# saptadeb/botLab

Measured on AMD Instinct MI355X. Metric: SLAM steps/sec (map+MCL+A*), higher is better.
Workload: dtype int8 grid / f32 poses with f64 intermediates / int64 weights; 1 GPU; full SLAM step on 200x200 @5cm grid (continuing from the shipped, already built obstacle_slam_10mx10m_5cm map), 100000 particles, 290 rays, A* replan on; particles=100000, rays=290, pipeline_depth=14, planner_lanes=2, planner_batch=6, parallelism=single GPU, collective=none

## Files before the change

### botlab_amd/csrc/bl_mcl.hip

```cpp
#include <math.h>
#include <stdio.h>
#include <stdlib.h>
#include <string.h>
#include <new>

#include <hip/hip_ext.h>
#include "bl_internal.h"
#include "bl_mcl_finish.h"

#define MCL_LDS_RAYS 384
#define MCL_MIN_BLOCKS 512
#define MCL_WIN_SMALL_BYTES (64 * 1024)
#define MCL_WIN_MAX 208
#define MCL_WIN_MARGIN 24
#define SCAN_THREADS 256
#define SCAN_ITEMS 2
#define SCAN_TILE (SCAN_THREADS * SCAN_ITEMS)


struct bl_pf {
    bl_ctx* ctx;
    int N, lo, hi, n_local;
    float4* rec[2];
    bool rec_external;
    int cur;
    double* tile_partials;
    ss_rec* fin_recs;
    ss_wild* fin_wild;
    int fin_subs_cap;
    mclf_tab_elem* fin_tabs;
    unsigned long long* fin_sync;
    unsigned int fin_gen;
    int fin_last_nrec;
    unsigned long long* prefix;
    float4* parent;
    pf_state* state;
    double* partials;
    int partials_cap;
    bool use_lds;
    int last_blocks, last_tile;
    int last_main_blocks, last_main_particles, last_tail_tile;
    bool fused_finish, no_fused_finish, no_packed, no_balance, no_framed, no_window, no_fast_trig, no_mirror_reuse, no_stage_dma, no_stage_x4;
    int window_override;
    int cus;
    int split_log2_override;
    int block_override;
    bool debug;
    bool strict;
    void* strict_recs; double* strict_starts;
    bool uniform_now;
    bool prefix_is_strict;
    double w_floor;
    unsigned long long* block_sums;
    int scan_blocks;
    int32_t* dbg_idx;
    int32_t* dbg_like;
    float* d_noise;
    bl_particle_t* d_export;
    int64_t pose_utime, parent_utime;
    bl_pose_xyt_t prev_odom;
    bool action_initialized, moved;
    double rot1, trans, rot2, rot1Std, transStd, rot2Std;
    uint64_t noise_seed;
    uint32_t step;
    bool initialized;
    bool pending_end;
    int64_t pending_utime;
// ... 313 lines not shown
    const pf_state* state;
    float4* parent;
    double* partials;
    int32_t* dbg_idx;
    int32_t* dbg_like;
    const int8_t* cells;
    const int8_t* framed;
    int framed_stride;
    bl_frame frame;
    const float* ranges;
    const float* thetas;
    const int64_t* times;
    int64_t t_begin; double t_den;
    int R;
    int N, lo, n_local;
    double r;
    double M_inv;
    double rot1, trans, rot2, rot1Std, transStd, rot2Std;
    const float* noise;
    uint32_t seed_lo, seed_hi, step;
    int interp;
    int resample;
    int strict;
    int win_w, win_h;
    int split_log2;
    int pk_ok;
    int theta_simple;
    int fast_trig;
    int stage_dma;
    float max_range_cells;
    int main_blocks, main_particles;
    const struct mcl_shard_tab* sh;
    struct pf_recovery_dev* rc;
};
struct mcl_shard_tab { int world, block; const float4* src[BL_MAX_SHARDS]; const unsigned long long* prefix[BL_MAX_SHARDS]; };

struct pf_recovery_dev {
    double w_slow, w_fast, w_avg, p;
    uint32_t updates, primed;
    unsigned long long t;
    unsigned long long total_at_fold;
    unsigned long long injected_total;
    const uint32_t* list;
    uint32_t F, W, k0, k1;
    double ox, oy, mpc;
};
#define RC_CTR 0x72637679u

__device__ __forceinline__ float4 gl_pose(const uint32_t a[4], uint32_t b0, const uint32_t* list, uint32_t F, uint32_t W,
                                          double ox, double oy, double mpc)
{
    const uint32_t r = (uint32_t)__umul64hi(((unsigned long long)a[0] << 32) | a[1], (unsigned long long)F);
    const uint32_t cell = list[r];
    const uint32_t cx = cell % W, cy = cell / W;
    const double fx = (double)(a[2] >> 8) * 0x1p-24, fy = (double)(a[3] >> 8) * 0x1p-24, ft = (double)(b0 >> 8) * 0x1p-24;
    const float x = (float)(ox + ((double)cx + fx) * mpc);
    const float y = (float)(oy + ((double)cy + fy) * mpc);
    const float th = bl_wrap_to_pi((float)((2.0 * ft - 1.0) * BL_PI));
    return make_float4(x, y, th, __uint_as_float(1u));
}

__device__ __forceinline__ float4 mcl_src_at(const mcl_args& a, int i)
{
    if (a.sh) return a.sh->src[i / a.sh->block][i];
    return a.src[i];
}
// ... 32 lines not shown
            float sn, cs;                                                               \
            bl_sincosf_cells(wrap_to_pi_cells(pth_r - rt.y, theta_simple), &sn, &cs);                   \
            acc += SCORE_EXPR;                                                          \
        }                                                                               \
    } while (0)

#define MCL_RAY_LOOP_FAST_RANGE(PM, LO, HI, HW)                                         \
    do {                                                                                \
        const int rounds_ = ((HI) - (LO)) >> sl2;                                       \
        int off_ = ((LO) + sub) * 16;                                                   \
        for (int k_ = 0; k_ < rounds_; ++k_, off_ += split * 16) {                      \
            const float4 rt = *(const float4*)((const char*)s_ray + off_);              \
            short2_t E_, X_;                                                            \
            ray_cells_fast<HW>(start, a.frame.cpm, rt.x, pth_r, rt.y, pcs_, rt.z, rt.w, trig_k1, trig_kh2, E_, X_);   \
            acc += score_cells_pk(PM, S, E_, X_);                                       \
        }                                                                               \
        if ((off_ >> 4) < (HI)) {                                                       \
            const float4 rt = *(const float4*)((const char*)s_ray + off_);              \
            short2_t E_, X_;                                                            \
            ray_cells_fast<HW>(start, a.frame.cpm, rt.x, pth_r, rt.y, pcs_, rt.z, rt.w, trig_k1, trig_kh2, E_, X_);   \
            acc += score_cells_pk(PM, S, E_, X_);                                       \
        }                                                                               \
    } while (0)
#define MCL_RAY_LOOP_FAST(PM) do { if (hw_trig_) MCL_RAY_LOOP_FAST_RANGE(PM, 0, cnt, true); else MCL_RAY_LOOP_FAST_RANGE(PM, 0, cnt, false); } while (0)

__device__ __forceinline__ double readlane_f64(double v, int lane)
{
    const int lo = __builtin_amdgcn_readlane(__double2loint(v), lane), hi = __builtin_amdgcn_readlane(__double2hiint(v), lane);
    return __hiloint2double(hi, lo);
}

__device__ __forceinline__ int kary_pos(int lo, int hi, int step, int k) { return min(lo + (k + 1) * step - 1, hi); }

__device__ __forceinline__ bool resample_reaches(double T, unsigned long long v, bool strict)
{
    return strict ? T <= __longlong_as_double((long long)v) : T <= (double)v;
}

#define MCL_BRACKET_Q 1
#define MCL_BRACKET_WINDOW 64
template <int Q, class Prefix>
__device__ __forceinline__ void resample_bracket(const Prefix& prefix, int N, double T, bool active,
                                                 int lane, int* out_lo, int* out_hi, bool strict = false, int m = -1)
{
    *out_lo = 0; *out_hi = N - 1;
    const unsigned long long act = __builtin_amdgcn_ballot_w64(active);
    if (!act) return;
    const double T0 = readlane_f64(T, __ffsll((long long)act) - 1), T1 = readlane_f64(T, 63 - __clzll((long long)act));
    const int m0 = __builtin_amdgcn_readlane(m, __ffsll((long long)act) - 1);
    if (m0 >= 0) {
        const int g = m0 - 31 * MCL_BRACKET_WINDOW;
        if (g >= 0 && g + 63 * MCL_BRACKET_WINDOW < N) {
            const unsigned long long v = prefix[g + lane * MCL_BRACKET_WINDOW];
            const unsigned long long b0 = __builtin_amdgcn_ballot_w64(resample_reaches(T0, v, strict));
            const unsigned long long b1 = __builtin_amdgcn_ballot_w64(resample_reaches(T1, v, strict));
            if (b0 && !(b0 & 1ull) && b1) {
                const int f0 = __ffsll((long long)b0) - 1, f1 = __ffsll((long long)b1) - 1;
                *out_lo = g + (f0 - 1) * MCL_BRACKET_WINDOW + 1;
                *out_hi = g + f1 * MCL_BRACKET_WINDOW;
                return;
            }
        }
    }
    int lo0 = 0, hi0 = N - 1, lo1 = 0, hi1 = N - 1;
    for (int round = 0; round < 8 && (lo0 < hi0 || lo1 < hi1); ++round) {
        const int step0 = (hi0 - lo0 + 64 * Q) / (64 * Q), step1 = (hi1 - lo1 + 64 * Q) / (64 * Q);
        unsigned long long v0[Q], v1[Q];
#pragma unroll
        for (int u = 0; u < Q; ++u) {
            v0[u] = prefix[kary_pos(lo0, hi0, step0, 64 * u + lane)];
            v1[u] = prefix[kary_pos(lo1, hi1, step1, 64 * u + lane)];
        }
        int f0 = -1, f1 = -1;
#pragma unroll
        for (int u = Q - 1; u >= 0; --u) {
            const unsigned long long b0 = __builtin_amdgcn_ballot_w64(resample_reaches(T0, v0[u], strict));
            const unsigned long long b1 = __builtin_amdgcn_ballot_w64(resample_reaches(T1, v1[u], strict));
            if (b0) f0 = 64 * u + __ffsll((long long)b0) - 1;
            if (b1) f1 = 64 * u + __ffsll((long long)b1) - 1;
        }
        if (f0 < 0) lo0 = hi0;
        else { const int nl = f0 ? kary_pos(lo0, hi0, step0, f0 - 1) + 1 : lo0; hi0 = kary_pos(lo0, hi0, step0, f0); lo0 = nl; }
        if (f1 < 0) lo1 = hi1;
        else { const int nl = f1 ? kary_pos(lo1, hi1, step1, f1 - 1) + 1 : lo1; hi1 = kary_pos(lo1, hi1, step1, f1); lo1 = nl; }
    }
    if (lo0 == hi0 && lo1 == hi1) { *out_lo = lo0; *out_hi = lo1; }
}
template <class Prefix>
__device__ __forceinline__ void resample_bracket(const Prefix& prefix, int N, double T, bool active,
                                                 int lane, int* out_lo, int* out_hi, bool strict = false, int m = -1)
{
    resample_bracket<1>(prefix, N, T, active, lane, out_lo, out_hi, strict, m);
}

template <class Prefix>
__device__ __forceinline__ int resample_bisect(const Prefix& prefix, double T, int lo, int hi, bool strict = false)
{
    while (lo < hi) {
        const int mid = (lo + hi) >> 1;
        if (resample_reaches(T, prefix[mid], strict)) hi = mid; else lo = mid + 1;
    }
    return lo;
}

#define MCL_STAGE_ROWS 6
template <class SrcRow>
__device__ __forceinline__ void stage_rows(int* s_map32, int rows, int wq, int q_lo, int q_hi, int sw, int n_sw, int lane, SrcRow src_row)
{
    for (int q0 = 0; q0 < wq; q0 += 64) {
        const int q = q0 + lane;
        const bool qin = q < wq, qdata = q >= q_lo && q < q_hi;
        for (int r0 = sw; r0 < rows; r0 += n_sw * MCL_STAGE_ROWS) {
            int v[MCL_STAGE_ROWS];
#pragma unroll
            for (int u = 0; u < MCL_STAGE_ROWS; ++u) {
                const int ry = r0 + u * n_sw;
                v[u] = 0;
                if (ry < rows) {
                    const int* src = src_row(ry);
                    if (src != nullptr && qdata) v[u] = src[q - q_lo];
                }
            }
#pragma unroll
            for (int u = 0; u < MCL_STAGE_ROWS; ++u) {
                const int ry = r0 + u * n_sw;
                if (ry < rows && qin) s_map32[ry * wq + q] = v[u];
            }
        }
    }
}

#ifdef MCL_STAMPS
#define MCL_STAMP_SLOTS 12
__device__ unsigned long long g_mcl_stamps[4096 * MCL_STAMP_SLOTS];
#define MCL_STAMP(k) do { if (threadIdx.x == 0 && blockIdx.x < 4096) g_mcl_stamps[blockIdx.x * MCL_STAMP_SLOTS + (k)] = wall_clock64(); } while (0)
// ... 127 lines not shown
            const int wq = win.w >> 2, fq = a.framed_stride >> 2;
            const int* f32 = (const int*)(a.framed - MCL_FRAME * a.framed_stride - 4);
            const int* org = f32 + (size_t)(win.y0 + MCL_FRAME) * fq + ((win.x0 + 4) >> 2);
            if (wq <= 64 && a.stage_dma) {
                if (lane < wq)
                    for (int ry = sw; ry < win.h; ry += n_sw)
                        __builtin_amdgcn_global_load_lds((const __attribute__((address_space(1))) void*)(org + (size_t)ry * fq + lane),
                                                         (__attribute__((address_space(3))) void*)(s_map32 + ry * wq), 4, 0, 0);
            } else
            stage_rows(s_map32, win.h, wq, 0, wq, sw, n_sw, lane, [&](int ry) -> const int* { return org + (size_t)ry * fq; });
        }
    }

    MCL_STAMP_T(4, pw * 64);
#ifdef MCL_STAMPS
    if (wave >= pw) { asm volatile("s_waitcnt vmcnt(0)" ::: "memory"); }
    MCL_STAMP_T(9, pw * 64);
#endif
    double t_units = 0, t_x = 0, t_y = 0, t_s = 0, t_c = 0;
    float2 pcs_own = make_float2(2.0f, 0.0f);
    float pth_sin = 0.0f, pth_cos = 1.0f;
    int i = mp;
    bool injected = false;
    float4 s = make_float4(0.f, 0.f, 0.f, 0.f);
    float px = 0.f, py = 0.f, pth = 0.f, sx0 = 0.f, sy0 = 0.f;
    double rs_T = 0.0;
    int rs_lo = 0, rs_hi = a.N - 1;
    const mcl_prefix_view pview = {a.sh, a.prefix};
    const int uni_n = a.resample ? a.state->uni_n : 0;
    if (a.resample && (!shared_pro || wave < pw)) {
        if (pro_active) { rs_T = a.r + mp * a.M_inv; if (!a.strict && uni_n <= 0) rs_T *= a.state->S; }
        if (uni_n > 0) { }
        else if (a.sh) resample_bracket(pview, a.N, rs_T, pro_active, lane, &rs_lo, &rs_hi, a.strict != 0);
        else resample_bracket<MCL_BRACKET_Q>(a.prefix, a.N, rs_T, pro_active, lane, &rs_lo, &rs_hi, a.strict != 0, pro_active ? mp : -1);
    }
    MCL_STAMP(5);
    if (pro_active) {
        if (a.resample && uni_n > 0) i = uni_search(a.state, uni_n, rs_T, a.N);
        else if (a.resample) i = a.sh ? resample_bisect(pview, rs_T, rs_lo, rs_hi, a.strict != 0) : resample_bisect(a.prefix, rs_T, rs_lo, rs_hi, a.strict != 0);
        MCL_STAMP(6);
        if (REC) {
            const pf_recovery_dev& rc = *a.rc;
            uint32_t d[4];
            bl_philox4x32((uint32_t)mp, rc.updates, RC_CTR, 2u, rc.k0, rc.k1, d);
            injected = (unsigned long long)d[0] < rc.t;
            if (injected) {
                uint32_t w0[4], w1[4];
                bl_philox4x32((uint32_t)mp, rc.updates, RC_CTR, 0u, rc.k0, rc.k1, w0);
                bl_philox4x32((uint32_t)mp, rc.updates, RC_CTR, 1u, rc.k0, rc.k1, w1);
                s = gl_pose(w0, w1[0], rc.list, rc.F, rc.W, rc.ox, rc.oy, rc.mpc);
                i = -1;
            }
        }
        if (!injected)
        s = mcl_src_at(a, i);
        float n1, n2, n3;
        if (a.noise) {
            n1 = a.noise[3 * jp]; n2 = a.noise[3 * jp + 1]; n3 = a.noise[3 * jp + 2];
        } else {
            float z[3];
            philox_normals3((uint32_t)mp, a.step, a.seed_lo, a.seed_hi, z);
            n1 = (float)(a.rot1 + a.rot1Std * (double)z[0]);
            n2 = (float)(a.trans + a.transStd * (double)z[1]);
            n3 = (float)(a.rot2 + a.rot2Std * (double)z[2]);
        }
        const float head = s.z + n1;
// ... 496 lines not shown
    if (t >= (long long)n_local * 12) return;
    const int j = (int)(t / 12), d = (int)(t % 12);
    uint32_t v;
    if (d < 5) {
        const float4 r = rec[lo + j];
        v = d == 0 ? (uint32_t)((uint64_t)pose_utime >> 32) : d == 1 ? (uint32_t)pose_utime
          : __float_as_uint(d == 2 ? r.x : (d == 3 ? r.y : r.z));
    } else if (d < 10) {
        const float4 p = parent[j];
        v = d == 5 ? (uint32_t)((uint64_t)parent_utime >> 32) : d == 6 ? (uint32_t)parent_utime
          : __float_as_uint(d == 7 ? p.x : (d == 8 ? p.y : p.z));
    } else {
        const double w = (double)__float_as_uint(rec[lo + j].w) / state->S;
        const uint64_t b = (uint64_t)__double_as_longlong(w);
        v = d == 10 ? (uint32_t)(b >> 32) : (uint32_t)b;
    }
    out[t] = bl_bswap32(v);
}

__global__ void k_pf_set_pose(pf_state* state, bl_pose_xyt_t pose, int only_utime)
{
    if (only_utime) state->pose.utime = pose.utime;
    else state->pose = pose;
}

static int pf_alloc(bl_pf* pf)
{
    size_t N = pf->cap, n = pf->cap_local;
    if (!pf->rec[0]) {
        BL_HIP(hipMalloc((void**)&pf->rec[0], N * sizeof(float4)));
        BL_HIP(hipMalloc((void**)&pf->rec[1], N * sizeof(float4)));
    }
    BL_HIP(hipMalloc((void**)&pf->prefix, N * sizeof(unsigned long long)));
    BL_HIP(hipMalloc((void**)&pf->parent, n * sizeof(float4)));
    BL_HIP(hipMalloc((void**)&pf->state, sizeof(pf_state)));
    int blocks = (int)((n * 64 + 255) / 256) + 1;
    BL_HIP(hipMalloc((void**)&pf->partials, (size_t)blocks * 5 * sizeof(double)));
    pf->partials_cap = blocks;
    static bool attr_set = false;
    if (!attr_set) {
        const int big = 384 * 384;
        BL_HIP(hipFuncSetAttribute((const void*)k_mcl_main<0, 256, 2>, hipFuncAttributeMaxDynamicSharedMemorySize, big));
        BL_HIP(hipFuncSetAttribute((const void*)k_mcl_main<0, 512, 2>, hipFuncAttributeMaxDynamicSharedMemorySize, big));
        BL_HIP(hipFuncSetAttribute((const void*)k_mcl_main<0, 1024, 2>, hipFuncAttributeMaxDynamicSharedMemorySize, big));
        BL_HIP(hipFuncSetAttribute((const void*)k_mcl_finish, hipFuncAttributeMaxDynamicSharedMemorySize, MCLF_LDS_BYTES));
        attr_set = true;
    }
    pf->scan_blocks = (int)((N + SCAN_TILE - 1) / SCAN_TILE);
    BL_HIP(hipMalloc((void**)&pf->block_sums, (size_t)pf->scan_blocks * sizeof(unsigned long long)));
    BL_HIP(hipMalloc((void**)&pf->tile_partials, (size_t)pf->scan_blocks * 5 * sizeof(double)));
    pf->fin_subs_cap = (int)(N / MCLF_SUB) + 4 * (MCLF_WG / 64);
    BL_HIP(hipMalloc((void**)&pf->fin_recs, (size_t)2 * pf->fin_subs_cap * sizeof(ss_rec)));
    if (!getenv("BOTLAB_MCL_NO_WILD")) BL_HIP(hipMalloc((void**)&pf->fin_wild, (size_t)2 * pf->fin_subs_cap * sizeof(ss_wild)));
    BL_HIP(hipMalloc((void**)&pf->fin_tabs, (size_t)2 * MCLF_TSLOTS * MCLF_SUB * sizeof(mclf_tab_elem)));
    BL_HIP(hipMalloc((void**)&pf->fin_sync, MCLF_SYNC_WORDS * sizeof(unsigned long long)));
    BL_HIP(hipMemsetAsync(pf->fin_sync, 0, MCLF_SYNC_WORDS * sizeof(unsigned long long), pf->ctx->stream));
    BL_HIP(hipMalloc((void**)&pf->dbg_idx, n * sizeof(int32_t)));
    BL_HIP(hipMalloc((void**)&pf->dbg_like, n * sizeof(int32_t)));
    BL_HIP(hipMemsetAsync(pf->dbg_idx, 0, n * sizeof(int32_t), pf->ctx->stream));
    BL_HIP(hipMemsetAsync(pf->dbg_like, 0, n * sizeof(int32_t), pf->ctx->stream));
    BL_HIP(hipMemsetAsync(pf->state, 0, sizeof(pf_state), pf->ctx->stream));
    return BL_OK;
}

extern "C" int bl_pf_create(bl_ctx* ctx, int num_particles, int shard_lo, int shard_hi, bl_pf** out)
{
    BL_CHECK_ARG(ctx != nullptr && out != nullptr);
    BL_CHECK_ARG(num_particles > 1);
    BL_CHECK_ARG(shard_lo >= 0 && shard_lo < shard_hi && shard_hi <= num_particles);
    BL_HIP(hipSetDevice(ctx->device));
    bl_pf* pf = new bl_pf();
    memset((void*)pf, 0, sizeof(*pf));
    pf->ctx = ctx;
    pf->N = num_particles; pf->lo = shard_lo; pf->hi = shard_hi; pf->n_local = shard_hi - shard_lo;
    pf->cap = num_particles; pf->cap_local = pf->n_local; pf->ad_next = num_particles;
    {
        volatile double wsum = 0.0;
        for (int i = 0; i < num_particles; ++i) wsum = wsum + 0.001;
        pf->w_floor = 0.001 / wsum;
    }
    pf->noise_seed = 0x243F6A8885A308D3ull;
    pf->use_lds = getenv("BOTLAB_MCL_NO_LDS") == nullptr;
    pf->no_fused_finish = getenv("BOTLAB_MCL_NO_FUSED_FINISH") != nullptr;
    pf->no_packed = getenv("BOTLAB_MCL_NO_PACKED") != nullptr;
    pf->no_balance = getenv("BOTLAB_MCL_NO_BALANCE") != nullptr;
    pf->no_framed = getenv("BOTLAB_MCL_NO_FRAMED") != nullptr;
    pf->no_mirror_reuse = getenv("BOTLAB_MCL_NO_MIRROR_REUSE") != nullptr;
    pf->no_stage_dma = getenv("BOTLAB_MCL_NO_STAGE_DMA") != nullptr;
    pf->no_stage_x4 = getenv("BOTLAB_MCL_NO_STAGE_X4") != nullptr;
    pf->no_window = getenv("BOTLAB_MCL_NO_WINDOW") != nullptr;
    pf->no_fast_trig = getenv("BOTLAB_MCL_NO_FAST_TRIG") != nullptr;
    pf->window_override = getenv("BOTLAB_MCL_WINDOW") ? atoi(getenv("BOTLAB_MCL_WINDOW")) : 0;
    { int cus = 0; if (hipDeviceGetAttribute(&cus, hipDeviceAttributeMultiprocessorCount, ctx->device) == hipSuccess) pf->cus = cus; }
    pf->split_log2_override = getenv("BOTLAB_MCL_SPLIT_LOG2") ? atoi(getenv("BOTLAB_MCL_SPLIT_LOG2")) : -1;
    if (pf->split_log2_override > 6) pf->split_log2_override = 6;
    pf->block_override = getenv("BOTLAB_MCL_BLOCK") ? atoi(getenv("BOTLAB_MCL_BLOCK")) : 0;
    if (pf->block_override != 0 && pf->block_override != 256 && pf->block_override != 512 && pf->block_override != 1024) pf->block_override = 0;
    *out = pf;
    return BL_OK;
}

extern "C" void bl_pf_destroy(bl_pf* pf)
{
    if (!pf) return;
    (void)hipStreamSynchronize(pf->ctx->stream);
    if (!pf->rec_external) { if (pf->rec[0]) (void)hipFree(pf->rec[0]); if (pf->rec[1]) (void)hipFree(pf->rec[1]); }
    void* ptrs[] = {pf->fin_wild, pf->tile_partials, pf->fin_recs, pf->fin_tabs, pf->fin_sync, pf->prefix, pf->parent, pf->state, pf->partials, pf->block_sums, pf->dbg_idx, pf->dbg_like,
                    pf->d_noise, pf->d_export, pf->sh_xchg, pf->sh_tab, pf->sh_fin, pf->sh_flags, pf->sh_peers_dev, pf->strict_recs, pf->strict_starts,
                    pf->gl_tiles, pf->gl_list, pf->sp_parts, pf->sp_out, pf->rc_list, pf->rc_dev, pf->ad_table};
    for (void* p : ptrs) if (p) (void)hipFree(p);
    if (pf->ad_hcount) { (void)hipHostFree(pf->ad_hcount); (void)hipEventDestroy(pf->ad_ev); }
    delete pf->ad_wfloor;
    delete pf;
}

extern "C" int bl_pf_set_exchange_buffers(bl_pf* pf, void* d_rec0, void* d_rec1)
{
    BL_CHECK_ARG(pf != nullptr && d_rec0 && d_rec1);
    if (pf->prefix) { bl_set_error("exchange buffers must be set before the filter is initialised"); return BL_ERR_STATE; }
    pf->rec[0] = (float4*)d_rec0; pf->rec[1] = (float4*)d_rec1; pf->rec_external = true;
    return BL_OK;
}

extern "C" void* bl_pf_exchange_rec_ptr(bl_pf* pf) { return pf && pf->prefix ? (void*)pf->rec[pf->pending_end ? pf->cur ^ 1 : pf->cur] : nullptr; }
extern "C" const void* bl_pf_pose_device_ptr(bl_pf* pf) { return pf && pf->state ? (const void*)&pf->state->pose : nullptr; }

static double pf_w_floor(const bl_pf* pf)
{
    return (pf->N == pf->cap || !pf->ad_wfloor) ? pf->w_floor : (*pf->ad_wfloor)[pf->N];
}

static void pf_adaptive_fill(bl_pf* pf)
{
    if (pf->ad_pending) { (void)hipEventSynchronize(pf->ad_ev); pf->ad_pending = false; }
    pf->ad_next = pf->cap;
    if (pf->N == pf->cap) return;
    pf->N = pf->n_local = pf->hi = pf->cap;
    pf->scan_blocks = (pf->cap + SCAN_TILE - 1) / SCAN_TILE;
}

// ... 25 lines not shown
        }
    }
    hipLaunchKernelGGL(k_pf_cumulative_strict, dim3(1), dim3(64), 0, pf->ctx->stream, pf->rec[which], pf->N, pf->state, (double*)pf->prefix);
}

static int pf_finish_fill(bl_pf* pf, mcl_finish_args* f)
{
    if (f->tile <= 0 || f->tail_tile <= 0) return -1;
    f->gthreads = mclf_gthreads(pf->N);
    for (int attempt = 0; attempt < 2; ++attempt) {
        const int chunk = mclf_chunk(f->gthreads);
        if (f->tile <= chunk && (chunk % f->tile) == 0 && f->tail_tile <= chunk && (chunk % f->tail_tile) == 0) break;
        if (attempt == 1 || f->gthreads == MCLF_GT_LARGE) return -1;
        f->gthreads = MCLF_GT_LARGE;
    }
    const int groups = mclf_groups(*f);
    f->groups = groups;
    f->groups_wait = groups;
    if (((++pf->fin_gen) & 0xffu) == 0u) ++pf->fin_gen;
    f->tag = pf->fin_gen;
    const int nrec = groups * (f->gthreads >> 6);
    if (pf->sh_world <= 1 && nrec != pf->fin_last_nrec && (int64_t)nrec <= pf->fin_subs_cap) {
        if (hipMemsetAsync(pf->fin_recs, 0, (size_t)2 * pf->fin_subs_cap * sizeof(ss_rec), pf->ctx->stream) != hipSuccess) return -1;
        pf->fin_last_nrec = nrec;
    }
    f->sh = nullptr;
    f->uni_mode = pf_uni_mode(pf, false);
    f->w_floor = pf_w_floor(pf);
    f->wild = pf->sh_world > 1 ? nullptr : pf->fin_wild;
    f->no_trees = getenv("BOTLAB_MCL_NO_TREES") != nullptr ? 1 : 0;
    f->recs = pf->fin_recs;
    f->tabs = pf->fin_tabs;
    f->sync = pf->fin_sync;
    if (pf->sh_world > 1) return groups;
    if ((int64_t)groups * (f->gthreads >> 6) > pf->fin_subs_cap) return -1;
    return groups;
}

static int pf_scan(bl_pf* pf, int which, int write_pose, int64_t utime)
{
    bl_ctx* ctx = pf->ctx;
    hipEvent_t e0, e1;
    int rc = bl_timer_begin(ctx, BL_K_MCL_SCAN, &e0, &e1);
    if (rc) return rc;
    hipLaunchKernelGGL(k_scan_tile_sums, dim3(pf->scan_blocks), dim3(SCAN_THREADS), 0, ctx->stream, pf->rec[which], pf->N,
                       pf->block_sums, write_pose ? pf->tile_partials : (double*)nullptr);
    if (write_pose) {
        mcl_finish_args f;
        f.partials = pf->tile_partials; f.nblocks = pf->scan_blocks;
        f.rec = pf->rec[which]; f.N = pf->N;
        f.tile = SCAN_TILE; f.main_blocks = pf->scan_blocks; f.main_particles = pf->N; f.tail_tile = 1;
        f.prefix = pf->prefix; f.state = pf->state; f.utime = utime;
        const int groups = pf_finish_fill(pf, &f);
        if (groups < 0) { bl_set_error("internal: finish launch shape"); return BL_ERR_STATE; }
        hipLaunchKernelGGL(k_mcl_finish, dim3(MCLF_EXTRA_WGS + f.groups_wait), dim3(MCLF_WG), MCLF_LDS_BYTES, ctx->stream, f);
    } else {
        hipLaunchKernelGGL(k_scan_write_prefix, dim3(pf->scan_blocks), dim3(SCAN_THREADS), 0, ctx->stream, pf->rec[which], pf->N,
                           pf->block_sums, pf->scan_blocks, pf->prefix, pf->state, pf_uni_mode(pf, true), pf_w_floor(pf));
    }
    BL_HIP(hipGetLastError());
    pf_strict_cumulative(pf, which);
    return bl_timer_end(ctx, BL_K_MCL_SCAN, e0, e1);
}

static void pf_reset_action(bl_pf* pf)
{
    pf->action_initialized = false; pf->moved = false;
    pf->rot1 = pf->trans = pf->rot2 = 0;
    pf->step = 0;
    pf->pending_end = false;
}

extern "C" int bl_pf_init_at_pose(bl_pf* pf, const bl_pose_xyt_t* pose, uint64_t seed)
{
    BL_CHECK_ARG(pf != nullptr && pose != nullptr);
    BL_HIP(hipSetDevice(pf->ctx->device));
    if (!pf->prefix) { int rc = pf_alloc(pf); if (rc) return rc; }
    pf_adaptive_fill(pf);
    pf->cur = 0;
    if (pf->sh_broken) { pf->sh_broken = false; BL_HIP(hipMemsetAsync(&pf->state->shard_broken, 0, sizeof(unsigned int), pf->ctx->stream)); }
    hipLaunchKernelGGL(k_pf_init, dim3((pf->N + 255) / 256), dim3(256), 0, pf->ctx->stream, pf->rec[0], pf->parent, pf->N,
                       pf->lo, pf->n_local, *pose, (uint32_t)seed, (uint32_t)(seed >> 32));
    hipLaunchKernelGGL(k_pf_set_pose, dim3(1), dim3(1), 0, pf->ctx->stream, pf->state, *pose, 0);
    BL_HIP(hipGetLastError());
    pf->pose_utime = pose->utime; pf->parent_utime = pose->utime;
    pf->initialized = true;
    pf->uniform_now = true;
    pf->sensed = false;
    return pf_scan(pf, 0, 0, 0);
}

// ... 254 lines not shown
    bl_ctx* ctx = pf->ctx;
    int n_out = pf->n_local;
    const bool resize = resample != 0 && (pf->ad_on || pf->N != pf->cap);
    if (resize) {
        int rc_a = pf_adaptive_resolve(pf);
        if (rc_a) return rc_a;
        n_out = pf->ad_next;
    }
    if (noise) { int rc_n = pf_upload_noise(pf, noise, n_out); if (rc_n) return rc_n; }
    mcl_args a;
    a.src = pf->rec[pf->cur];
    a.dst = pf->rec[pf->cur ^ 1];
    a.prefix = pf->prefix;
    a.state = pf->state;
    a.parent = pf->parent;
    a.partials = pf->partials;
    a.dbg_idx = pf->debug ? pf->dbg_idx : nullptr; a.dbg_like = pf->debug ? pf->dbg_like : nullptr;
    a.cells = map ? map->cells : nullptr;
    if (map) a.frame = map->frame; else memset(&a.frame, 0, sizeof(a.frame));
    a.ranges = ctx->scan.ranges; a.thetas = ctx->scan.thetas; a.times = ctx->scan.times;
    a.t_begin = pf->pose_utime; a.t_den = (pf->pose_utime != 0) ? (double)(0 - pf->pose_utime) : 1.0;
    a.R = R;
    a.N = pf->N; a.lo = pf->lo; a.n_local = n_out;
    a.M_inv = 1.0 / (resize ? n_out : pf->N);
    a.r = (((double)rand_value) / (double)RAND_MAX) * a.M_inv;
    a.rot1 = pf->rot1; a.trans = pf->trans; a.rot2 = pf->rot2;
    a.rot1Std = pf->rot1Std; a.transStd = pf->transStd; a.rot2Std = pf->rot2Std;
    a.noise = noise ? pf->d_noise : nullptr;
    a.seed_lo = (uint32_t)pf->noise_seed; a.seed_hi = (uint32_t)(pf->noise_seed >> 32);
    a.step = pf->step;
    a.resample = resample;
    a.strict = pf->prefix_is_strict ? 1 : 0;
    if (getenv("BOTLAB_MCL_DIAG_NOSEARCH")) a.resample = 0;
    a.interp = (map && pf->pose_utime != 0) ? 1 : 0;
    a.theta_simple = ctx->scan.thetas_simple ? 1 : 0;
    a.max_range_cells = map ? ctx->scan.max_range * a.frame.cpm : 0.0f;
    static const bool hw_trig = getenv("BOTLAB_MCL_HW_TRIG") != nullptr;
    a.fast_trig = (a.theta_simple && !pf->no_fast_trig) ? (hw_trig ? 2 : 1) : 0;
    a.stage_dma = pf->no_stage_dma ? 0 : 1;
    a.pk_ok = (map && a.frame.width <= 8192 && a.frame.height <= 8192 && ctx->scan.max_range * a.frame.cpm <= 4000.0f &&
               !pf->no_packed) ? 1 : 0;
    int lds_bytes = 0, mode = 0;
    a.win_w = 0; a.win_h = 0;
    a.framed = nullptr; a.framed_stride = 0;
    if (map) {
        const int W = map->frame.width, H = map->frame.height;
        const int stride = ((W + 3) & ~3) + 8;
        const size_t whole = (size_t)stride * (H + 2 * MCL_FRAME);
        auto ensure_mirror = [&]() -> int {
            if (whole > map->mirror_cap) {
                if (map->mirror) { BL_HIP(hipStreamSynchronize(ctx->stream)); BL_HIP(hipFree(map->mirror)); map->mirror = nullptr; map->mirror_cap = 0; }
                BL_HIP(hipMalloc((void**)&map->mirror, whole));
                map->mirror_cap = whole;
                map->mirror_valid = false;
            }
            if (!map->mirror_valid || map->mirror_stride != stride || map->mirror_external || pf->no_mirror_reuse) {
                const int dwords = (stride >> 2) * (H + 2 * MCL_FRAME);
                hipLaunchKernelGGL(k_mcl_frame, dim3((dwords + 255) / 256), dim3(256), 0, ctx->stream, map->cells, W, H, stride, (int*)map->mirror);
                map->mirror_stride = stride;
                map->mirror_valid = map->ctx == ctx;
            }
            a.framed = map->mirror + MCL_FRAME * stride + 4;
            a.framed_stride = stride;
            return BL_OK;
        };
        if (pf->use_lds && whole <= MCL_WIN_SMALL_BYTES) {
// ... 1327 lines not shown
```

### botlab_amd/csrc/bl_mcl_finish.h

```cpp
#ifndef BL_MCL_FINISH_H
#define BL_MCL_FINISH_H

#include "bl_internal.h"
#include "bl_serial_sum.h"

#define UNI_MAX 192
struct uni_seg { double c0, inc, last; int i0, n; };

struct pf_state {
    double S;
    bl_pose_xyt_t pose;
    unsigned int wait_timeouts;
    unsigned int shard_broken;
    double sums_used[5];
    unsigned int chain_stats[8];
    unsigned int lookahead[2];
    unsigned int pre_stats[2];
    unsigned long long cstamps[16];
    unsigned long long gstamps[8];
    unsigned long long stamps[6];
    int uni_n;
    int uni_pad;
    uni_seg uni[UNI_MAX];
    unsigned long long xstamps[16];
// ... 1 lines not shown

struct mclf_tab_elem { double t; int se, se1; };

#define BL_MAX_SHARDS 8
#define MCLF_XCHG_HDR 64
struct mclf_shards {
    int world;
    int rank;
    int block;
    int subs_per_rank;
    const float4* rec[BL_MAX_SHARDS];
    char* xchg;
    size_t xchg_stride;
};

struct mcl_finish_args {
    const double* partials; int nblocks;
    const float4* rec; int N;
    int tile, main_blocks, main_particles, tail_tile;
    unsigned long long* prefix;
    pf_state* state;
    int64_t utime;
    int uni_mode;
    double w_floor;
    ss_rec* recs;
    mclf_tab_elem* tabs;
    unsigned long long* sync;
    int groups, gthreads;
    ss_wild* wild;
    int groups_wait;
    unsigned int tag;
    const mclf_shards* sh;
    int no_trees;
};

#define MCLF_POSE_THREADS 256
#define MCLF_WG 1024
#define MCLF_ITEMS 2
#define MCLF_SUB (64 * MCLF_ITEMS)
#define MCLF_GT_SMALL 256
#define MCLF_GT_LARGE 1024
#define MCLF_GT_SWITCH 160000
#define MCLF_RISKY 0x1000
#define MCLF_WILD 0x2000
#define MCLF_TSLOT_SHIFT 16
#define MCLF_KEY_MASK 0xfff
#define MCLF_MARGIN 4096
#define MCLF_TSLOTS 20
#define MCLF_MAXENT 32
#define MCLF_PRE_SUBS 9
#define MCLF_EXTRA_WGS 2
#define MCLF_PRE_STEPPED 2
#define MCLF_TAB_WAVES 4
#define MCLF_SPIN_LIMIT (1u << 20)
#define MCLF_SYNC_WORDS 8
#define MCLF_LDS_BYTES (112 * 1024)

static inline int mclf_gthreads(int N) { return N >= MCLF_GT_SWITCH ? MCLF_GT_LARGE : MCLF_GT_SMALL; }
#define mclf_chunk(gthreads) ((gthreads) * MCLF_ITEMS)

static inline int mclf_groups(const mcl_finish_args& f)
{
    const int chunk = mclf_chunk(f.gthreads);
    const int tpc_main = chunk / f.tile;
    const int tail_blocks = f.nblocks - f.main_blocks;
    int g = (f.main_blocks + tpc_main - 1) / tpc_main;
// ... 39 lines not shown
        c = tail + w;
    }
    *last_out = c;
    return (fits || !seg) ? ns : 0;
}

__device__ inline int uni_search(const pf_state* st, int uni_n, double T, int N)
{
    int lo = 0, hi = uni_n - 1;
    while (lo < hi) { const int mid = (lo + hi) >> 1; if (st->uni[mid].last >= T) hi = mid; else lo = mid + 1; }
    const uni_seg s_ = st->uni[lo];
    if (!(s_.last >= T)) return N - 1;
    if (T <= s_.c0 || s_.n <= 1) return s_.i0;
    long long k = (long long)((T - s_.c0) / s_.inc);
    if (k < 0) k = 0;
    if (k > s_.n - 1) k = s_.n - 1;
    while (k < s_.n - 1 && s_.c0 + (double)k * s_.inc < T) ++k;
    while (k > 0 && s_.c0 + (double)(k - 1) * s_.inc >= T) --k;
    return s_.i0 + (int)k;
}

__device__ inline void uni_update(pf_state* st, int N, double S, int mode, double w_floor)
{
    int n = 0;
    if (mode >= 0) {
        double w = 0.0, last;
        if (mode == 1) w = 1.0 / (double)N;
        else if (S == 2.0 * (double)N) w = w_floor;
        if (w > 0.0) n = uni_build(w, N, st->uni, UNI_MAX, &last);
    }
    st->uni_n = n;
}

#define MCLF_MAXW (MCLF_WG / 64)
struct mclf_smem {
    unsigned long long off[MCLF_MAXW], wave[MCLF_MAXW], tot[MCLF_MAXW];
    double bx[MCLF_MAXW], by[MCLF_MAXW];
    double wx[MCLF_MAXW], wy[MCLF_MAXW];
    double red[MCLF_POSE_THREADS / 64][5];
    float xy[2], first[2];
    unsigned int stats[8];
    int tbase[2][BL_MAX_SHARDS + 1];
    int ntab_seen[2];
    double pre[2][MCLF_PRE_STEPPED * MCLF_SUB];
    double psum[2][MCLF_PRE_SUBS];
    ss_wild pmap[2][MCLF_PRE_SUBS];
};

#ifdef MCLF_STAMPS
#define MCLF_NOW() ((unsigned long long)wall_clock64())
#else
#define MCLF_NOW() 0ull
#endif

__device__ __forceinline__ double mclf_wave_sum(double v)
{
    for (int off = 32; off > 0; off >>= 1) v += __shfl_down(v, off, 64);
    return v;
}
__device__ __forceinline__ double mclf_wave_sum_all(double v)
{
    for (int off = 32; off > 0; off >>= 1) v += __shfl_xor(v, off, 64);
    return v;
}

__device__ __forceinline__ void mclf_store_u64(unsigned long long* p, unsigned long long v)
// ... 290 lines not shown
        const int Mp = ss_mag((float)predicted_start);
        risky = anybad || !(Mp + lo - MCLF_MARGIN > SS_MLO && Mp + hi + MCLF_MARGIN < SS_MHI);
        rec = anybad ? ss_rec_make(MCLF_RISKY, 0, 0, 0) : ss_rec_make(key | (risky ? MCLF_RISKY : 0), D, lo, hi);
        up_only = !anybad && Mp + lo > SS_MLO && Mp + hi + MCLF_MARGIN < 2 * SS_MHI && (key & 0xff) < 254;
    }
    const bool dirty = risky && f.wild != nullptr && key != 0;
    bool got_table = false;
    if (risky && f.tabs && (!dirty || up_only)) {
        unsigned long long got = 0;
        if (lane == 0) got = __hip_atomic_fetch_add(mclf_tab_counter(f), axis ? (1ull << 16) : 1ull, __ATOMIC_RELAXED, __HIP_MEMORY_SCOPE_AGENT);
        const int slot = __builtin_amdgcn_readfirstlane((int)((got >> (axis ? 16 : 0)) & 0xffffull));
        if (slot < MCLF_TSLOTS) {
            int p1[MCLF_ITEMS] = {0, 0}, bad1[MCLF_ITEMS] = {1, 1};
            const bool up = key != 0 && (key & 0xff) < 254;
            if (up) mclf_prefix_in(key + 1, t, cnt, p1, bad1);
            mclf_tab_elem* tab = mclf_tab_ptr(f, axis, f.sh ? f.sh->rank : 0, slot);
#pragma unroll
            for (int k = 0; k < MCLF_ITEMS; ++k) {
                const int se = key ? ((p[k] << 1) | bad[k]) : 1, se1 = up ? ((p1[k] << 1) | bad1[k]) : 1;
                mclf_store_tab(tab + lane * MCLF_ITEMS + k, t[k], se, se1);
            }
            rec.key |= (slot + 1) << MCLF_TSLOT_SHIFT;
            got_table = slot < MCLF_TSLOTS / 2;
        }
    }
    if (dirty && !got_table) {
        have_wild = mclf_build_wild(f, axis, t, cnt, predicted_start, key, lane, sub_index);
        if (have_wild && !up_only) return ss_rec_make(MCLF_RISKY | MCLF_WILD, 0, 0, 0);
    }
    if (have_wild && (rec.key & MCLF_RISKY)) rec.key |= MCLF_WILD;
    return rec;
}

__device__ __forceinline__ void mclf_prefix_group(const mcl_finish_args& f, int g, mclf_smem& sm)
{
    const int tid = threadIdx.x, lane = tid & 63, wave = tid >> 6;
    if (tid >= f.gthreads) return;
    const int gt = f.gthreads, nw = gt >> 6;
#ifdef MCLF_STAMPS
    unsigned long long gs[8] = {MCLF_NOW(), 0, 0, 0, 0, 0, 0, 0};
#define MCLF_GSTAMP(i) gs[i] = MCLF_NOW()
#else
#define MCLF_GSTAMP(i) do { } while (0)
#endif
    int first_block, lo, hi;
    mclf_group_range(f, g, &first_block, &lo, &hi);
    const int base = lo + tid * MCLF_ITEMS;
    float4 r[MCLF_ITEMS];
    int cnt = 0;
#pragma unroll
    for (int k = 0; k < MCLF_ITEMS; ++k) {
        r[k] = make_float4(0.f, 0.f, 0.f, 0.f);
        if (base + k < hi) { r[k] = f.rec[base + k]; cnt = k + 1; }
    }
    unsigned long long before = 0, total = 0;
    double bx = 0.0, by = 0.0;
    for (int j0 = tid; j0 < f.nblocks; j0 += 4 * gt) {
        double pu[4], px4[4], py4[4];
#pragma unroll
        for (int q = 0; q < 4; ++q) {
            const int j = j0 + q * gt;
            const size_t at = (size_t)(j < f.nblocks ? j : 0) * 5;
            pu[q] = f.partials[at]; px4[q] = f.partials[at + 1]; py4[q] = f.partials[at + 2];
        }
#pragma unroll
        for (int q = 0; q < 4; ++q) {
// ... 2 lines not shown
                const unsigned long long u = (unsigned long long)pu[q];
                total += u;
                if (j < first_block) { before += u; bx += px4[q]; by += py4[q]; }
            }
        }
    }
#ifdef MCLF_STAMPS
    asm volatile("s_waitcnt vmcnt(0)" ::: "memory");
    if (tid == 0 && g == f.groups / 2) f.state->xstamps[0] = MCLF_NOW();
#endif
    for (int off = 32; off > 0; off >>= 1) { before += __shfl_xor(before, off, 64); total += __shfl_xor(total, off, 64); }
    bx = mclf_wave_sum_all(bx); by = mclf_wave_sum_all(by);
    if (lane == 0) { sm.off[wave] = before; sm.tot[wave] = total; sm.bx[wave] = bx; sm.by[wave] = by; }
    unsigned long long loc[MCLF_ITEMS];
    unsigned long long run = 0;
#pragma unroll
    for (int k = 0; k < MCLF_ITEMS; ++k) { run += __float_as_uint(r[k].w); loc[k] = run; }
    unsigned long long incl = run;
    for (int off = 1; off < 64; off <<= 1) {
        unsigned long long t = __shfl_up(incl, off, 64);
        if (lane >= off) incl += t;
    }
    if (lane == 63) sm.wave[wave] = incl;
    MCLF_GSTAMP(1);
    __syncthreads();
    MCLF_GSTAMP(2);
    unsigned long long off0 = incl - run, S_u = 0;
    double px = 0.0, py = 0.0;
    for (int w = 0; w < nw; ++w) { off0 += sm.off[w]; S_u += sm.tot[w]; px += sm.bx[w]; py += sm.by[w]; if (w < wave) off0 += sm.wave[w]; }
    if (!f.recs) {
#pragma unroll
        for (int k = 0; k < MCLF_ITEMS; ++k)
            if (base + k < hi) f.prefix[base + k] = off0 + loc[k];
        return;
    }
    MCLF_GSTAMP(3);
    const double S = (double)S_u;
    const double St = mclf_term_S(f, S);
    double tx[MCLF_ITEMS], ty[MCLF_ITEMS];
    double sx = 0.0, sy = 0.0;
#pragma unroll
    for (int k = 0; k < MCLF_ITEMS; ++k) {
        tx[k] = mclf_term(r[k], St, 0); ty[k] = mclf_term(r[k], St, 1);
        sx += tx[k]; sy += ty[k];
    }
    sx = mclf_wave_sum_all(sx); sy = mclf_wave_sum_all(sy);
    if (lane == 0) { sm.wx[wave] = sx; sm.wy[wave] = sy; }
    MCLF_GSTAMP(4);
    __syncthreads();
    px /= S; py /= S;
    for (int w = 0; w < wave; ++w) { px += sm.wx[w]; py += sm.wy[w]; }
    const bool very_first = g * nw + wave < MCLF_PRE_SUBS;
    const ss_rec rx = mclf_make_record(f, 0, tx, cnt, px, very_first, lane, g * nw + wave);
    const ss_rec ry = mclf_make_record(f, 1, ty, cnt, py, very_first, lane, g * nw + wave);
    MCLF_GSTAMP(5);
    const bool side_data = (rx.key != SS_ID && (rx.key & MCLF_RISKY) != 0) || (ry.key != SS_ID && (ry.key & MCLF_RISKY) != 0);
    if (side_data) mclf_drain_stores();
    if (lane == 0) {
        const int s = g * nw + wave;
        mclf_store_rec(mclf_rec_ptr(f, 0, s), rx, f.tag);
        mclf_store_rec(mclf_rec_ptr(f, 1, s), ry, f.tag);
    }
#pragma unroll
    for (int k = 0; k < MCLF_ITEMS; ++k)
        if (base + k < hi) f.prefix[base + k] = off0 + loc[k];
    MCLF_GSTAMP(6);
#ifdef MCLF_STAMPS
    if (tid == 0 && g == f.groups / 2) { gs[7] = MCLF_NOW(); for (int k = 0; k < 8; ++k) f.state->gstamps[k] = gs[k]; }
#endif
}

__device__ __forceinline__ double mclf_readlane_f64(double v, int lane)
{
    const int lo = __builtin_amdgcn_readlane(__double2loint(v), lane), hi = __builtin_amdgcn_readlane(__double2hiint(v), lane);
    return __hiloint2double(hi, lo);
}

__device__ __forceinline__ float mclf_replay(const double (&t)[MCLF_ITEMS], int n, int pos, int head, float acc, int lane, unsigned int* phases,
                                             double* lds_terms = nullptr)
{
    static_assert(MCLF_ITEMS == 2, "the replay indexes two terms per lane");
    n = __builtin_amdgcn_readfirstlane(n); pos = __builtin_amdgcn_readfirstlane(pos); head = __builtin_amdgcn_readfirstlane(head);
    if (pos < head) {
        const int h = min(head, n);
        if (lds_terms) {
            *(double2*)&lds_terms[2 * lane] = make_double2(t[0], t[1]);
            asm volatile("s_waitcnt lgkmcnt(0)" ::: "memory");
#pragma unroll 8
            for (int i = pos; i < h; ++i) acc = ss_exact_step(acc, lds_terms[i]);
        } else {
#pragma unroll 8
            for (int i = pos; i < h; ++i) acc = ss_exact_step(acc, mclf_readlane_f64((i & 1) ? t[1] : t[0], i >> 1));
        }
        pos = h;
    }
    int budget = 4;
    while (pos < n) {
        const int key = __builtin_amdgcn_readfirstlane(ss_key(acc));
// ... 974 lines not shown
```

Before: 12250 steps/s.

## Precompute resample index table in finish kernel to skip prefix bracket search

The fused finish kernel now writes a table mapping each systematic-resample target index to its source particle, computed from the inclusive prefix sums, tagged with a generation byte. The MCL kernel reads two table entries per particle instead of running the ballot-based bracket search over the prefix array, and falls back to the search if tags mismatch or validation fails. This replaces a multi-step dependent global search with a direct lookup. In exchange it adds an extra N+1 word table written each step, per-lane fill loops in the finish kernel, and one validating prefix read.

Measured after the change: 12410 steps/s (median of 6 runs). +1.3%, better.

```diff
diff --git a/botlab_amd/csrc/bl_mcl.hip b/botlab_amd/csrc/bl_mcl.hip
--- a/botlab_amd/csrc/bl_mcl.hip
+++ b/botlab_amd/csrc/bl_mcl.hip
@@ -33,6 +33,10 @@
     unsigned int fin_gen;
     int fin_last_nrec;
     unsigned long long* prefix;
+    uint32_t* rs_tab;
+    unsigned int rs_tag;
+    int rs_tab_n;
+    bool no_rs_table;
     float4* parent;
     pf_state* state;
     double* partials;
@@ -412,6 +416,8 @@
     int main_blocks, main_particles;
     const struct mcl_shard_tab* sh;
     struct pf_recovery_dev* rc;
+    const uint32_t* rs_tab;
+    unsigned int rs_tag;
 };
 struct mcl_shard_tab { int world, block; const float4* src[BL_MAX_SHARDS]; const unsigned long long* prefix[BL_MAX_SHARDS]; };
 
@@ -510,10 +516,6 @@
 
 __device__ __forceinline__ int kary_pos(int lo, int hi, int step, int k) { return min(lo + (k + 1) * step - 1, hi); }
 
-__device__ __forceinline__ bool resample_reaches(double T, unsigned long long v, bool strict)
-{
-    return strict ? T <= __longlong_as_double((long long)v) : T <= (double)v;
-}
 
 #define MCL_BRACKET_Q 1
 #define MCL_BRACKET_WINDOW 64
@@ -579,6 +581,25 @@
         if (resample_reaches(T, prefix[mid], strict)) hi = mid; else lo = mid + 1;
     }
     return lo;
+}
+
+__device__ __forceinline__ void resample_from_table(const unsigned long long* prefix, const uint32_t* tab, unsigned int tag, int N, double T,
+                                                    bool active, int m, int lane, int* out_lo, int* out_hi)
+{
+    bool ok = true;
+    int lo = 0, hi = N - 1;
+    if (active) {
+        const uint32_t e0 = tab[m], e1 = tab[m + 1];
+        const uint32_t tg = tag & 0xffu;
+        lo = (int)(e0 & RS_IDX_MASK); hi = (int)(e1 & RS_IDX_MASK);
+        ok = (e0 >> RS_IDX_BITS) == tg && (e1 >> RS_IDX_BITS) == tg && lo <= hi && hi < N;
+        if (ok && hi != N - 1) ok = resample_reaches(T, prefix[hi], false);
+    }
+    if (__builtin_amdgcn_ballot_w64(!ok)) {
+        resample_bracket<MCL_BRACKET_Q>(prefix, N, T, active, lane, out_lo, out_hi, false, active ? m : -1);
+        return;
+    }
+    *out_lo = lo; *out_hi = hi;
 }
 
 #define MCL_STAGE_ROWS 6
@@ -772,6 +793,7 @@
         if (pro_active) { rs_T = a.r + mp * a.M_inv; if (!a.strict && uni_n <= 0) rs_T *= a.state->S; }
         if (uni_n > 0) { }
         else if (a.sh) resample_bracket(pview, a.N, rs_T, pro_active, lane, &rs_lo, &rs_hi, a.strict != 0);
+        else if (a.rs_tab) resample_from_table(a.prefix, a.rs_tab, a.rs_tag, a.N, rs_T, pro_active, mp, lane, &rs_lo, &rs_hi);
         else resample_bracket<MCL_BRACKET_Q>(a.prefix, a.N, rs_T, pro_active, lane, &rs_lo, &rs_hi, a.strict != 0, pro_active ? mp : -1);
     }
     MCL_STAMP(5);
@@ -1334,6 +1356,9 @@
         BL_HIP(hipMalloc((void**)&pf->rec[1], N * sizeof(float4)));
     }
     BL_HIP(hipMalloc((void**)&pf->prefix, N * sizeof(unsigned long long)));
+    BL_HIP(hipMalloc((void**)&pf->rs_tab, (N + 1) * sizeof(uint32_t)));
+    BL_HIP(hipMemsetAsync(pf->rs_tab, 0, (N + 1) * sizeof(uint32_t), pf->ctx->stream));
+    pf->rs_tag = 0;
     BL_HIP(hipMalloc((void**)&pf->parent, n * sizeof(float4)));
     BL_HIP(hipMalloc((void**)&pf->state, sizeof(pf_state)));
     int blocks = (int)((n * 64 + 255) / 256) + 1;
@@ -1392,6 +1417,7 @@
     pf->no_stage_x4 = getenv("BOTLAB_MCL_NO_STAGE_X4") != nullptr;
     pf->no_window = getenv("BOTLAB_MCL_NO_WINDOW") != nullptr;
     pf->no_fast_trig = getenv("BOTLAB_MCL_NO_FAST_TRIG") != nullptr;
+    pf->no_rs_table = getenv("BOTLAB_MCL_NO_RS_TABLE") != nullptr;
     pf->window_override = getenv("BOTLAB_MCL_WINDOW") ? atoi(getenv("BOTLAB_MCL_WINDOW")) : 0;
     { int cus = 0; if (hipDeviceGetAttribute(&cus, hipDeviceAttributeMultiprocessorCount, ctx->device) == hipSuccess) pf->cus = cus; }
     pf->split_log2_override = getenv("BOTLAB_MCL_SPLIT_LOG2") ? atoi(getenv("BOTLAB_MCL_SPLIT_LOG2")) : -1;
@@ -1407,7 +1433,7 @@
     if (!pf) return;
     (void)hipStreamSynchronize(pf->ctx->stream);
     if (!pf->rec_external) { if (pf->rec[0]) (void)hipFree(pf->rec[0]); if (pf->rec[1]) (void)hipFree(pf->rec[1]); }
-    void* ptrs[] = {pf->fin_wild, pf->tile_partials, pf->fin_recs, pf->fin_tabs, pf->fin_sync, pf->prefix, pf->parent, pf->state, pf->partials, pf->block_sums, pf->dbg_idx, pf->dbg_like,
+    void* ptrs[] = {pf->fin_wild, pf->tile_partials, pf->fin_recs, pf->fin_tabs, pf->fin_sync, pf->prefix, pf->rs_tab, pf->parent, pf->state, pf->partials, pf->block_sums, pf->dbg_idx, pf->dbg_like,
                     pf->d_noise, pf->d_export, pf->sh_xchg, pf->sh_tab, pf->sh_fin, pf->sh_flags, pf->sh_peers_dev, pf->strict_recs, pf->strict_starts,
                     pf->gl_tiles, pf->gl_list, pf->sp_parts, pf->sp_out, pf->rc_list, pf->rc_dev, pf->ad_table};
     for (void* p : ptrs) if (p) (void)hipFree(p);
@@ -1499,6 +1525,11 @@
     f->recs = pf->fin_recs;
     f->tabs = pf->fin_tabs;
     f->sync = pf->fin_sync;
+    const bool rs = !pf->no_rs_table && pf->sh_world <= 1 && pf->N < (int)RS_IDX_MASK;
+    f->rs_tab = rs ? pf->rs_tab : nullptr;
+    f->rs_minv = 1.0 / pf->N;
+    pf->rs_tag = rs ? f->tag : 0u;
+    pf->rs_tab_n = pf->N;
     if (pf->sh_world > 1) return groups;
     if ((int64_t)groups * (f->gthreads >> 6) > pf->fin_subs_cap) return -1;
     return groups;
@@ -1524,6 +1555,7 @@
     } else {
         hipLaunchKernelGGL(k_scan_write_prefix, dim3(pf->scan_blocks), dim3(SCAN_THREADS), 0, ctx->stream, pf->rec[which], pf->N,
                            pf->block_sums, pf->scan_blocks, pf->prefix, pf->state, pf_uni_mode(pf, true), pf_w_floor(pf));
+        pf->rs_tag = 0;
     }
     BL_HIP(hipGetLastError());
     pf_strict_cumulative(pf, which);
@@ -1844,6 +1876,11 @@
     a.resample = resample;
     a.strict = pf->prefix_is_strict ? 1 : 0;
     if (getenv("BOTLAB_MCL_DIAG_NOSEARCH")) a.resample = 0;
+    a.rs_tab = nullptr; a.rs_tag = 0;
+    if (a.resample && !a.strict && pf->sh_world <= 1 && pf->rs_tag != 0 && pf->rs_tab_n == pf->N && (resize ? n_out : pf->N) == pf->N) {
+        a.rs_tab = pf->rs_tab; a.rs_tag = pf->rs_tag;
+    }
+    pf->rs_tag = 0;
     a.interp = (map && pf->pose_utime != 0) ? 1 : 0;
     a.theta_simple = ctx->scan.thetas_simple ? 1 : 0;
     a.max_range_cells = map ? ctx->scan.max_range * a.frame.cpm : 0.0f;
diff --git a/botlab_amd/csrc/bl_mcl_finish.h b/botlab_amd/csrc/bl_mcl_finish.h
--- a/botlab_amd/csrc/bl_mcl_finish.h
+++ b/botlab_amd/csrc/bl_mcl_finish.h
@@ -57,6 +57,8 @@
     unsigned int tag;
     const mclf_shards* sh;
     int no_trees;
+    uint32_t* rs_tab;
+    double rs_minv;
 };
 
 #define MCLF_POSE_THREADS 256
@@ -162,6 +164,52 @@
     st->uni_n = n;
 }
 
+#define RS_IDX_BITS 24
+#define RS_IDX_MASK ((1u << RS_IDX_BITS) - 1u)
+#define RS_LANE_RUN 4
+
+__device__ __forceinline__ bool resample_reaches(double T, unsigned long long v, bool strict)
+{
+    return strict ? T <= __longlong_as_double((long long)v) : T <= (double)v;
+}
+__device__ __forceinline__ double rs_target(int j, double minv, double S) { return ((double)j * minv) * S; }
+__device__ __forceinline__ int rs_first_above(unsigned long long P, double S, double minv, int M)
+{
+    long long e = (long long)((double)P / S * (double)M);
+    e = e < 0 ? 0 : e > M ? M : e;
+    while (e > 0 && !resample_reaches(rs_target((int)e - 1, minv, S), P, false)) --e;
+    while (e < M && resample_reaches(rs_target((int)e, minv, S), P, false)) ++e;
+    return (int)e;
+}
+__device__ __forceinline__ void rs_table_write(uint32_t* tab, unsigned int tag, int N, double S, double minv, int base, int cnt,
+                                               unsigned long long p_before, const unsigned long long (&p)[MCLF_ITEMS], int lane)
+{
+    const int M = N;
+    const uint32_t tg = (tag & 0xffu) << RS_IDX_BITS;
+    int j0[MCLF_ITEMS], j1[MCLF_ITEMS];
+    int jl = base == 0 ? 0 : rs_first_above(p_before, S, minv, M);
+#pragma unroll
+    for (int k = 0; k < MCLF_ITEMS; ++k) {
+        const int i = base + k;
+        j0[k] = jl;
+        j1[k] = k < cnt ? (i == N - 1 ? M + 1 : rs_first_above(p[k], S, minv, M)) : jl;
+        jl = j1[k];
+        if (j1[k] - j0[k] <= RS_LANE_RUN)
+            for (int j = j0[k]; j < j1[k]; ++j) tab[j] = (uint32_t)i | tg;
+    }
+#pragma unroll
+    for (int k = 0; k < MCLF_ITEMS; ++k) {
+        unsigned long long longs = __builtin_amdgcn_ballot_w64(j1[k] - j0[k] > RS_LANE_RUN);
+        while (longs) {
+            const int l = __ffsll((long long)longs) - 1;
+            longs &= longs - 1;
+            const int s = __builtin_amdgcn_readlane(j0[k], l), e = __builtin_amdgcn_readlane(j1[k], l);
+            const uint32_t v = (uint32_t)(__builtin_amdgcn_readlane(base, l) + k) | tg;
+            for (int j = s + lane; j < e; j += 64) tab[j] = v;
+        }
+    }
+}
+
 #define MCLF_MAXW (MCLF_WG / 64)
 struct mclf_smem {
     unsigned long long off[MCLF_MAXW], wave[MCLF_MAXW], tot[MCLF_MAXW];
@@ -518,6 +566,16 @@
     return rec;
 }
 
+__device__ __forceinline__ void mclf_rs_table(const mcl_finish_args& f, int base, int cnt, unsigned long long off0,
+                                              const unsigned long long (&loc)[MCLF_ITEMS], unsigned long long S_u, int lane)
+{
+    if (!f.rs_tab || S_u == 0) return;
+    unsigned long long p[MCLF_ITEMS];
+#pragma unroll
+    for (int k = 0; k < MCLF_ITEMS; ++k) p[k] = off0 + loc[k];
+    rs_table_write(f.rs_tab, f.tag, f.N, (double)S_u, f.rs_minv, base, cnt, off0, p, lane);
+}
+
 __device__ __forceinline__ void mclf_prefix_group(const mcl_finish_args& f, int g, mclf_smem& sm)
 {
     const int tid = threadIdx.x, lane = tid & 63, wave = tid >> 6;
@@ -586,6 +644,7 @@
 #pragma unroll
         for (int k = 0; k < MCLF_ITEMS; ++k)
             if (base + k < hi) f.prefix[base + k] = off0 + loc[k];
+        mclf_rs_table(f, base, cnt, off0, loc, S_u, lane);
         return;
     }
     MCLF_GSTAMP(3);
@@ -618,6 +677,7 @@
 #pragma unroll
     for (int k = 0; k < MCLF_ITEMS; ++k)
         if (base + k < hi) f.prefix[base + k] = off0 + loc[k];
+    mclf_rs_table(f, base, cnt, off0, loc, S_u, lane);
     MCLF_GSTAMP(6);
 #ifdef MCLF_STAMPS
     if (tid == 0 && g == f.groups / 2) { gs[7] = MCLF_NOW(); for (int k = 0; k < 8; ++k) f.state->gstamps[k] = gs[k]; }
```
